# adr-arroyo/PointCloudComparator

Measured on AMD Instinct MI355X. Metric: nn_queries_per_sec, higher is better.
Workload: dtype f32; 1 GPU; C3: 10M x 10M XYZRGB (32-B stride), k=1 NN; step = index build over 10000000 references + 10000000 queries on each GPU (10000000 over 1 GPU); backend=none, engine=grid, references=10000000, queries_per_gpu=10000000, queries_total=10000000, point_stride_bytes=32

## Files before the change

pointcloudcomparator_amd/csrc/cellsort_mp.hip:

```cpp
#include "pcc_internal.hpp"
#include "grid_device.hpp"
#include "lane_ops.hpp"

namespace pcc {

constexpr int MP_T = 256;
constexpr unsigned int MP_F2 = 2048;
constexpr unsigned int MP_B2 = 128;
constexpr unsigned int MP_MAX_B1 = 256;
constexpr unsigned int MP_MAX_G = 512;
constexpr unsigned int MP_SLICE2 = 8192;
constexpr unsigned int MP_STAGE_BYTES = 32768;
constexpr unsigned int MP_WIN = 8;
#ifndef PCC_MP_STAGE_PTS
#define PCC_MP_STAGE_PTS 3072
#endif
#ifndef PCC_MP_STAGE_ORD
#define PCC_MP_STAGE_ORD 6144
#endif
constexpr unsigned int MP_FINE_STAGE_PTS = PCC_MP_STAGE_PTS, MP_FINE_STAGE_ORD = PCC_MP_STAGE_ORD;

struct MpPlan {
    unsigned int F1, F2, B1, G1, slice1;
};
static MpPlan mp_plan(unsigned int ncells_cap, unsigned int n) {
    MpPlan p;
    p.F2 = MP_F2;
    while ((unsigned long long)p.F2 * MP_B2 * MP_MAX_B1 < (unsigned long long)ncells_cap + 1) p.F2 *= 2;
    p.F1 = p.F2 * MP_B2;
    p.B1 = (ncells_cap + p.F1) / p.F1;
    p.G1 = (n + 16383) / 16384;
    if (p.G1 > MP_MAX_G) p.G1 = MP_MAX_G;
    if (p.G1 < 1) p.G1 = 1;
    p.slice1 = (n + p.G1 - 1) / p.G1;
    return p;
}

__device__ __forceinline__ unsigned int mp_cell(const float4& v, const GridParams& g, bool voxel) {
    return voxel ? voxel_id(v, g) : cell_id(v, g);
}
__device__ __forceinline__ unsigned int mp_cell(const uint2& v, const GridParams&, bool) { return v.x; }
__device__ __forceinline__ unsigned int mp_position(const float4& v) { return (unsigned int)__float_as_int(v.w); }
__device__ __forceinline__ unsigned int mp_position(const uint2& v) { return v.y; }
template <class E> __device__ __forceinline__ E mp_make(const float4& v, unsigned int cell);
template <> __device__ __forceinline__ float4 mp_make<float4>(const float4& v, unsigned int) { return v; }
template <> __device__ __forceinline__ uint2 mp_make<uint2>(const float4& v, unsigned int cell) {
    return make_uint2(cell, (unsigned int)__float_as_int(v.w));
}

__global__ void __launch_bounds__(MP_T)
k_mp_hist1(const float4* __restrict__ pts, unsigned int n, const GridDev* __restrict__ gd, unsigned int F1, unsigned int B1,
           unsigned int slice, unsigned int* __restrict__ H, unsigned int* __restrict__ zero, unsigned int n_zero) {
    for (unsigned int z = blockIdx.x * MP_T + threadIdx.x; z < n_zero; z += gridDim.x * MP_T) zero[z] = 0u;
    __shared__ unsigned int cnt[MP_MAX_B1];
    const GridParams g = gd->g;
    const bool voxel = gd->voxel != 0;
    for (unsigned int b = threadIdx.x; b < B1; b += MP_T) cnt[b] = 0;
    __syncthreads();
    const unsigned int beg = blockIdx.x * slice, end = min(n, beg + slice);
    for (unsigned int i0 = beg + threadIdx.x; i0 < end; i0 += 4 * MP_T) {
        float4 v[4];
#pragma unroll
        for (int u = 0; u < 4; ++u)
            if (i0 + u * MP_T < end) v[u] = pts[i0 + u * MP_T];
#pragma unroll
        for (int u = 0; u < 4; ++u)
            if (i0 + u * MP_T < end && __float_as_int(v[u].w) >= 0) atomicAdd(&cnt[mp_cell(v[u], g, voxel) / F1], 1u);
    }
    __syncthreads();
    for (unsigned int b = threadIdx.x; b < B1; b += MP_T) H[(size_t)b * gridDim.x + blockIdx.x] = cnt[b];
    if (blockIdx.x == 0 && threadIdx.x == 0) H[(size_t)B1 * gridDim.x] = 0;
}

template <class E>
__global__ void __launch_bounds__(MP_T)
k_mp_scatter1(const float4* __restrict__ pts, unsigned int n, const GridDev* __restrict__ gd, unsigned int F1, unsigned int B1,
              unsigned int slice, const unsigned int* __restrict__ H, E* __restrict__ out) {
    __shared__ unsigned int cur[MP_MAX_B1];
    const GridParams g = gd->g;
    const bool voxel = gd->voxel != 0;
    for (unsigned int b = threadIdx.x; b < B1; b += MP_T) cur[b] = H[(size_t)b * gridDim.x + blockIdx.x];
    __syncthreads();
    const unsigned int beg = blockIdx.x * slice, end = min(n, beg + slice);
    for (unsigned int i0 = beg + threadIdx.x; i0 < end; i0 += 4 * MP_T) {
        float4 v[4];
#pragma unroll
        for (int u = 0; u < 4; ++u)
            if (i0 + u * MP_T < end) v[u] = pts[i0 + u * MP_T];
#pragma unroll
        for (int u = 0; u < 4; ++u)
            if (i0 + u * MP_T < end && __float_as_int(v[u].w) >= 0) {
                const unsigned int c = mp_cell(v[u], g, voxel);
                out[atomicAdd(&cur[c / F1], 1u)] = mp_make<E>(v[u], c);
            }
    }
}

__global__ void __launch_bounds__(MP_T)
k_mp_hist1_cells(const unsigned int* __restrict__ cells, unsigned int n, unsigned int F1, unsigned int B1, unsigned int slice,
                 unsigned int* __restrict__ H, unsigned int* __restrict__ zero, unsigned int n_zero) {
    for (unsigned int z = blockIdx.x * MP_T + threadIdx.x; z < n_zero; z += gridDim.x * MP_T) zero[z] = 0u;
    __shared__ unsigned int cnt[MP_MAX_B1];
    for (unsigned int b = threadIdx.x; b < B1; b += MP_T) cnt[b] = 0;
    __syncthreads();
    const unsigned int beg = blockIdx.x * slice, end = min(n, beg + slice);
    for (unsigned int i0 = beg + threadIdx.x; i0 < end; i0 += 8 * MP_T) {
        unsigned int c[8];
#pragma unroll
        for (int u = 0; u < 8; ++u) c[u] = i0 + u * MP_T < end ? cells[i0 + u * MP_T] : 0xffffffffu;
#pragma unroll
        for (int u = 0; u < 8; ++u)
            if (c[u] != 0xffffffffu) atomicAdd(&cnt[c[u] / F1], 1u);
    }
    __syncthreads();
    for (unsigned int b = threadIdx.x; b < B1; b += MP_T) H[(size_t)b * gridDim.x + blockIdx.x] = cnt[b];
    if (blockIdx.x == 0 && threadIdx.x == 0) H[(size_t)B1 * gridDim.x] = 0;
}
__global__ void __launch_bounds__(MP_T)
k_mp_scatter1_cells(const unsigned int* __restrict__ cells, unsigned int n, unsigned int F1, unsigned int B1, unsigned int slice,
                    const unsigned int* __restrict__ H, uint2* __restrict__ out) {
    __shared__ unsigned int cur[MP_MAX_B1];
    for (unsigned int b = threadIdx.x; b < B1; b += MP_T) cur[b] = H[(size_t)b * gridDim.x + blockIdx.x];
    __syncthreads();
    const unsigned int beg = blockIdx.x * slice, end = min(n, beg + slice);
    for (unsigned int i0 = beg + threadIdx.x; i0 < end; i0 += 8 * MP_T) {
        unsigned int c[8];
#pragma unroll
        for (int u = 0; u < 8; ++u) c[u] = i0 + u * MP_T < end ? cells[i0 + u * MP_T] : 0xffffffffu;
#pragma unroll
        for (int u = 0; u < 8; ++u)
            if (c[u] != 0xffffffffu) out[atomicAdd(&cur[c[u] / F1], 1u)] = make_uint2(c[u], i0 + u * MP_T);
    }
}

constexpr unsigned int MP_TILE1 = 2048;
template <class E>
__global__ void __launch_bounds__(MP_T)
k_mp_scatter1_staged(const float4* __restrict__ pts, unsigned int n, const GridDev* __restrict__ gd, unsigned int F1, unsigned int B1,
                     unsigned int slice, const unsigned int* __restrict__ H, E* __restrict__ out) {
    constexpr int PER = MP_TILE1 / MP_T;
    __shared__ unsigned int cur[MP_MAX_B1], tcnt[MP_MAX_B1], tstart[MP_MAX_B1];
    __shared__ unsigned short sb[MP_TILE1];
    __shared__ __attribute__((aligned(16))) unsigned char stage_raw[MP_TILE1 * sizeof(E)];
    E* stage = reinterpret_cast<E*>(stage_raw);
    const GridParams g = gd->g;
    const bool voxel = gd->voxel != 0;
    for (unsigned int b = threadIdx.x; b < B1; b += MP_T) cur[b] = H[(size_t)b * gridDim.x + blockIdx.x];
    const unsigned int beg = blockIdx.x * slice, end = min(n, beg + slice);
    for (unsigned int t0 = beg; t0 < end; t0 += MP_TILE1) {
        for (unsigned int b = threadIdx.x; b < MP_MAX_B1; b += MP_T) tcnt[b] = 0;
        __syncthreads();
        float4 v[PER];
        unsigned int bk[PER], rk[PER];
#pragma unroll
        for (int u = 0; u < PER; ++u) {
            const unsigned int i = t0 + threadIdx.x + u * MP_T;
            v[u] = make_float4(0.f, 0.f, 0.f, __int_as_float(-1));
            if (i < end) v[u] = pts[i];
        }
#pragma unroll
        for (int u = 0; u < PER; ++u) {
            bk[u] = 0xffffffffu;
            rk[u] = 0;
            if (__float_as_int(v[u].w) >= 0) {
                bk[u] = mp_cell(v[u], g, voxel);
                rk[u] = atomicAdd(&tcnt[bk[u] / F1], 1u);
            }
        }
        __syncthreads();
        if (threadIdx.x < 64) {
            unsigned int c[4], sum = 0;
#pragma unroll
            for (int j = 0; j < 4; ++j) { c[j] = tcnt[4 * threadIdx.x + j]; sum += c[j]; }
            unsigned int ex = wave_incl_scan_add(sum) - sum;
#pragma unroll
            for (int j = 0; j < 4; ++j) { tstart[4 * threadIdx.x + j] = ex; ex += c[j]; }
        }
        __syncthreads();
#pragma unroll
        for (int u = 0; u < PER; ++u)
            if (bk[u] != 0xffffffffu) {
                const unsigned int b = bk[u] / F1, slot = tstart[b] + rk[u];
                stage[slot] = mp_make<E>(v[u], bk[u]);
                sb[slot] = (unsigned short)b;
            }
        __syncthreads();
        const unsigned int tile_n = tstart[MP_MAX_B1 - 1] + tcnt[MP_MAX_B1 - 1];
        for (unsigned int j = threadIdx.x; j < tile_n; j += MP_T) {
            const unsigned int b = sb[j];
            out[cur[b] + (j - tstart[b])] = stage[j];
        }
        __syncthreads();
        for (unsigned int b = threadIdx.x; b < MP_MAX_B1; b += MP_T) cur[b] += tcnt[b];
    }
}

__device__ __forceinline__ unsigned int mp_pair(unsigned int c, unsigned int F1, unsigned int F2) {
    return (c / F1) * MP_B2 + (c % F1) / F2;
}

template <bool PLACE, class E>
__global__ void __launch_bounds__(MP_T)
k_mp_level2(const E* __restrict__ in, const unsigned int* __restrict__ n_valid_ptr, const GridDev* __restrict__ gd,
            unsigned int F1, unsigned int F2, unsigned int* __restrict__ C, E* __restrict__ out) {
    constexpr unsigned int SLICE = PLACE ? MP_STAGE_BYTES / sizeof(E) : MP_SLICE2;
    __shared__ unsigned int cnt[MP_WIN * MP_B2];
    __shared__ __attribute__((aligned(16))) unsigned char stage_raw[PLACE ? MP_STAGE_BYTES : 16];
    E* stage = reinterpret_cast<E*>(stage_raw);
    const GridParams g = gd->g;
    const bool voxel = gd->voxel != 0;
    const unsigned int n = *n_valid_ptr;
    const unsigned int beg = blockIdx.x * SLICE, end = min(n, beg + SLICE);
    if (beg >= end) return;
    const unsigned int w0 = (mp_cell(in[beg], g, voxel) / F1) * MP_B2;
    for (unsigned int k = threadIdx.x; k < MP_WIN * MP_B2; k += MP_T) cnt[k] = 0;
    __syncthreads();
    for (unsigned int i0 = beg + threadIdx.x; i0 < end; i0 += 4 * MP_T) {
        E v[4];
#pragma unroll
        for (int u = 0; u < 4; ++u)
            if (i0 + u * MP_T < end) v[u] = in[i0 + u * MP_T];
#pragma unroll
        for (int u = 0; u < 4; ++u) {
            if (i0 + u * MP_T >= end) break;
            if (PLACE) stage[i0 + u * MP_T - beg] = v[u];
            const unsigned int pr = mp_pair(mp_cell(v[u], g, voxel), F1, F2);
            if (pr - w0 < MP_WIN * MP_B2) atomicAdd(&cnt[pr - w0], 1u);
            else if (!PLACE) atomicAdd(&C[pr], 1u);
            else out[atomicAdd(&C[pr], 1u)] = v[u];
        }
    }
    __syncthreads();
    for (unsigned int k = threadIdx.x; k < MP_WIN * MP_B2; k += MP_T) {
        const unsigned int c = cnt[k];
        if (c) {
            if (!PLACE) atomicAdd(&C[w0 + k], c);
            else cnt[k] = atomicAdd(&C[w0 + k], c);
        }
    }
    if (!PLACE) return;
    __syncthreads();
    for (unsigned int j = threadIdx.x; j < end - beg; j += MP_T) {
        const E v = stage[j];
        const unsigned int pr = mp_pair(mp_cell(v, g, voxel), F1, F2);
        if (pr - w0 < MP_WIN * MP_B2) out[atomicAdd(&cnt[pr - w0], 1u)] = v;
    }
}

__device__ __forceinline__ void mp_store_point(float4* out, unsigned int pos, const float4& v) { if (out) out[pos] = v; }
__device__ __forceinline__ void mp_store_point(float4*, unsigned int, const uint2&) {}

template <bool REFS, class E>
__global__ void __launch_bounds__(MP_T)
k_mp_fine(const E* __restrict__ in, const unsigned int* __restrict__ ends , const GridDev* __restrict__ gd,
          unsigned int F2, float4* __restrict__ out_pts, unsigned int* __restrict__ out_order,
          unsigned int* __restrict__ cell_start) {
    extern __shared__ __attribute__((aligned(16))) unsigned int lds[];
    unsigned int* cnt = lds;
    unsigned int* wsum = lds + F2;
    const GridParams g = gd->g;
    const bool voxel = gd->voxel != 0;
    const unsigned int ncells = (unsigned int)g.ncells;
    const unsigned int b = blockIdx.x;
    const unsigned int cell0 = b * F2;
    if (cell0 > ncells) return;
    const unsigned int beg = b ? ends[b - 1] : 0u, end = ends[b];
    if (!REFS && beg == end) return;
    for (unsigned int f = threadIdx.x; f < F2; f += MP_T) cnt[f] = 0;
    __syncthreads();
    for (unsigned int j0 = beg + threadIdx.x; j0 < end; j0 += 4 * MP_T) {
        E v[4];
#pragma unroll
        for (int u = 0; u < 4; ++u)
            if (j0 + u * MP_T < end) v[u] = in[j0 + u * MP_T];
#pragma unroll
        for (int u = 0; u < 4; ++u)
            if (j0 + u * MP_T < end) atomicAdd(&cnt[mp_cell(v[u], g, voxel) - cell0], 1u);
    }
    __syncthreads();
    const unsigned int per = (F2 + MP_T - 1) / MP_T;
    const unsigned int f0 = threadIdx.x * per, f1 = min(F2, f0 + per);
    unsigned int s = 0;
    for (unsigned int f = f0; f < f1; ++f) s += cnt[f];
    const unsigned int lane = threadIdx.x & 63, wave = threadIdx.x >> 6;
    const unsigned int inc = wave_incl_scan_add(s);
    if (lane == 63) wsum[wave] = inc;
    __syncthreads();
    unsigned int run = beg + inc - s;
    for (unsigned int w = 0; w < wave; ++w) run += wsum[w];
    for (unsigned int f = f0; f < f1; ++f) {
        const unsigned int c = cnt[f];
        cnt[f] = run;
        if (REFS && cell0 + f <= ncells) cell_start[cell0 + f] = run;
        run += c;
    }
    __syncthreads();
    const unsigned int stage_cap = out_pts ? MP_FINE_STAGE_PTS : MP_FINE_STAGE_ORD;
    const bool staged = end - beg <= stage_cap;
    float4* st_pts = reinterpret_cast<float4*>(lds + ((F2 + 4 + 3) & ~3u));
    unsigned int* st_ord = reinterpret_cast<unsigned int*>(st_pts + (out_pts ? MP_FINE_STAGE_PTS : 0));
    for (unsigned int j0 = beg + threadIdx.x; j0 < end; j0 += 4 * MP_T) {
        E v[4];
#pragma unroll
        for (int u = 0; u < 4; ++u)
            if (j0 + u * MP_T < end) v[u] = in[j0 + u * MP_T];
#pragma unroll
        for (int u = 0; u < 4; ++u) {
            if (j0 + u * MP_T >= end) break;
            const unsigned int pos = atomicAdd(&cnt[mp_cell(v[u], g, voxel) - cell0], 1u);
            if (staged) {
                mp_store_point(out_pts ? st_pts : nullptr, pos - beg, v[u]);
                if (out_order) st_ord[pos - beg] = mp_position(v[u]);
            } else {
                mp_store_point(out_pts, pos, v[u]);
                if (out_order) out_order[pos] = mp_position(v[u]);
            }
        }
    }
    if (staged) {
        __syncthreads();
        for (unsigned int i = threadIdx.x; i < end - beg; i += MP_T) {
            if (out_pts) out_pts[beg + i] = st_pts[i];
            if (out_order) out_order[beg + i] = st_ord[i];
        }
    }
}

int cell_sort_mp(pcc_index* ix, const float4* pts, size_t n_pts, bool refs, float4* out_pts, unsigned int* out_order,
                 unsigned int* cell_start, unsigned int** n_sorted_dev, const GridDev* gd_override,
                 unsigned int nc_cap_override) {
    hipStream_t s = ix->stream;
    const unsigned int n = (unsigned int)n_pts;
    const unsigned int ncap = gd_override ? nc_cap_override : ix->nc_cap;
    const MpPlan p = mp_plan(ncap, n);
    const GridDev* gd = gd_override ? gd_override : ix->d_grid.as<GridDev>();
    const unsigned int np = p.B1 * MP_B2;
    PCC_TRY(ix->mp_a.reserve((size_t)n * sizeof(float4) + 256));
    PCC_TRY(ix->mp_b.reserve((size_t)n * sizeof(float4) + 256));
    const size_t h_elems = (size_t)p.B1 * p.G1 + 1;
    PCC_TRY(ix->scratch_b.reserve(((h_elems + 3) & ~(size_t)3) * sizeof(unsigned int)));
    PCC_TRY(ix->mp_c.reserve(((size_t)np + 8) * sizeof(unsigned int)));
    unsigned int* H = ix->scratch_b.as<unsigned int>();
    unsigned int* C = ix->mp_c.as<unsigned int>();
    const unsigned int* cells = nullptr;
    if (!refs && !out_pts && !gd_override && pts == ix->q_packed.as<float4>() && ix->q_cells_n == n_pts && n_pts != 0)
        cells = ix->q_cells.as<unsigned int>();
    if (!refs) ix->q_cells_n = 0;
    if (cells)
        hipLaunchKernelGGL(k_mp_hist1_cells, dim3(p.G1), dim3(MP_T), 0, s, cells, n, p.F1, p.B1, p.slice1, H, C, np);
    else
    hipLaunchKernelGGL(k_mp_hist1, dim3(p.G1), dim3(MP_T), 0, s, pts, n, gd, p.F1, p.B1, p.slice1, H, C, np);
    PCC_HIP(hipGetLastError());
    PCC_TRY(launch_exclusive_scan(ix, s, H, h_elems, ix->scratch_a));
    unsigned int* n_valid = H + h_elems - 1;
    if (n_sorted_dev) *n_sorted_dev = n_valid;
    const size_t lds3 = (((size_t)p.F2 + 4 + 3) & ~(size_t)3) * sizeof(unsigned int) +
                        (out_pts ? (size_t)MP_FINE_STAGE_PTS * (sizeof(float4) + (out_order ? sizeof(unsigned int) : 0))
                                 : (size_t)MP_FINE_STAGE_ORD * sizeof(unsigned int));
    const unsigned int g2c = (n + MP_SLICE2 - 1) / MP_SLICE2;
    if (out_pts) {
        float4* t1 = ix->mp_a.as<float4>();
        float4* t2 = ix->mp_b.as<float4>();
        const unsigned int g2p = (n + MP_STAGE_BYTES / sizeof(float4) - 1) / (MP_STAGE_BYTES / sizeof(float4));
        if (ix->opt.sort_stage1)
            hipLaunchKernelGGL((k_mp_scatter1_staged<float4>), dim3(p.G1), dim3(MP_T), 0, s, pts, n, gd, p.F1, p.B1, p.slice1, H, t1);
        else
            hipLaunchKernelGGL((k_mp_scatter1<float4>), dim3(p.G1), dim3(MP_T), 0, s, pts, n, gd, p.F1, p.B1, p.slice1, H, t1);
        hipLaunchKernelGGL((k_mp_level2<false, float4>), dim3(g2c), dim3(MP_T), 0, s, t1, n_valid, gd, p.F1, p.F2, C, t2);
        PCC_TRY(launch_exclusive_scan(ix, s, C, np, ix->scratch_a));
        hipLaunchKernelGGL((k_mp_level2<true, float4>), dim3(g2p), dim3(MP_T), 0, s, t1, n_valid, gd, p.F1, p.F2, C, t2);
        if (refs)
            hipLaunchKernelGGL((k_mp_fine<true, float4>), dim3(np), dim3(MP_T), lds3, s, t2, C, gd, p.F2, out_pts, out_order, cell_start);
        else
            hipLaunchKernelGGL((k_mp_fine<false, float4>), dim3(np), dim3(MP_T), lds3, s, t2, C, gd, p.F2, out_pts, out_order, cell_start);
    } else {
        uint2* t1 = ix->mp_a.as<uint2>();
        uint2* t2 = ix->mp_b.as<uint2>();
        const unsigned int g2p = (n + MP_STAGE_BYTES / sizeof(uint2) - 1) / (MP_STAGE_BYTES / sizeof(uint2));
        if (cells)
            hipLaunchKernelGGL(k_mp_scatter1_cells, dim3(p.G1), dim3(MP_T), 0, s, cells, n, p.F1, p.B1, p.slice1, H, t1);
        else if (ix->opt.sort_stage1 == 2)
            hipLaunchKernelGGL((k_mp_scatter1_staged<uint2>), dim3(p.G1), dim3(MP_T), 0, s, pts, n, gd, p.F1, p.B1, p.slice1, H, t1);
        else
            hipLaunchKernelGGL((k_mp_scatter1<uint2>), dim3(p.G1), dim3(MP_T), 0, s, pts, n, gd, p.F1, p.B1, p.slice1, H, t1);
        hipLaunchKernelGGL((k_mp_level2<false, uint2>), dim3(g2c), dim3(MP_T), 0, s, t1, n_valid, gd, p.F1, p.F2, C, t2);
        PCC_TRY(launch_exclusive_scan(ix, s, C, np, ix->scratch_a));
        hipLaunchKernelGGL((k_mp_level2<true, uint2>), dim3(g2p), dim3(MP_T), 0, s, t1, n_valid, gd, p.F1, p.F2, C, t2);
        if (refs)
            hipLaunchKernelGGL((k_mp_fine<true, uint2>), dim3(np), dim3(MP_T), lds3, s, t2, C, gd, p.F2, out_pts, out_order, cell_start);
        else
            hipLaunchKernelGGL((k_mp_fine<false, uint2>), dim3(np), dim3(MP_T), lds3, s, t2, C, gd, p.F2, out_pts, out_order, cell_start);
    }
    PCC_HIP(hipGetLastError());
    return PCC_OK;
}

}
```

Measured before the change: 7.300 billion queries/s.

## Add wave-level and single-read paths for light buckets in fine cell sort

The fine cell-sort kernel now picks a path by bucket size. Buckets with at most `light` points are handled by one wave each, using 16-bit packed counters and a wave-local scan, with four such buckets per extra block. Mid-size buckets use a one-read block path that keeps points in registers and records each point's rank from the counting atomic, so the input is not read a second time. This is meant to cut per-bucket block overhead, barriers and repeated global reads on sparse buckets. The cost is extra blocks in the grid, more LDS reserved per block, and a lot more branching and code complexity.

```diff
diff --git a/pointcloudcomparator_amd/csrc/cellsort_mp.hip b/pointcloudcomparator_amd/csrc/cellsort_mp.hip
--- a/pointcloudcomparator_amd/csrc/cellsort_mp.hip
+++ b/pointcloudcomparator_amd/csrc/cellsort_mp.hip
@@ -1,6 +1,7 @@
 #include "pcc_internal.hpp"
 #include "grid_device.hpp"
 #include "lane_ops.hpp"
+#include <algorithm>
 
 namespace pcc {
 
@@ -251,21 +252,12 @@
 __device__ __forceinline__ void mp_store_point(float4*, unsigned int, const uint2&) {}
 
 template <bool REFS, class E>
-__global__ void __launch_bounds__(MP_T)
-k_mp_fine(const E* __restrict__ in, const unsigned int* __restrict__ ends , const GridDev* __restrict__ gd,
-          unsigned int F2, float4* __restrict__ out_pts, unsigned int* __restrict__ out_order,
-          unsigned int* __restrict__ cell_start) {
-    extern __shared__ __attribute__((aligned(16))) unsigned int lds[];
+__device__ __forceinline__ void mp_fine_block(unsigned int* lds, const E* __restrict__ in, unsigned int beg, unsigned int end, unsigned int cell0,
+                                              const GridParams& g, bool voxel, unsigned int F2, float4* __restrict__ out_pts,
+                                              unsigned int* __restrict__ out_order, unsigned int* __restrict__ cell_start) {
     unsigned int* cnt = lds;
     unsigned int* wsum = lds + F2;
-    const GridParams g = gd->g;
-    const bool voxel = gd->voxel != 0;
     const unsigned int ncells = (unsigned int)g.ncells;
-    const unsigned int b = blockIdx.x;
-    const unsigned int cell0 = b * F2;
-    if (cell0 > ncells) return;
-    const unsigned int beg = b ? ends[b - 1] : 0u, end = ends[b];
-    if (!REFS && beg == end) return;
     for (unsigned int f = threadIdx.x; f < F2; f += MP_T) cnt[f] = 0;
     __syncthreads();
     for (unsigned int j0 = beg + threadIdx.x; j0 < end; j0 += 4 * MP_T) {
@@ -323,6 +315,163 @@
             if (out_pts) out_pts[beg + i] = st_pts[i];
             if (out_order) out_order[beg + i] = st_ord[i];
         }
+    }
+}
+
+#ifndef PCC_MP_LIGHT_PTS
+#define PCC_MP_LIGHT_PTS 1024
+#endif
+#ifndef PCC_MP_LIGHT_ORD
+#define PCC_MP_LIGHT_ORD 1024
+#endif
+template <class E> struct MpWave;
+template <> struct MpWave<float4> {
+    typedef float4 Staged;
+    static constexpr unsigned int LIGHT = PCC_MP_LIGHT_PTS;
+    static __device__ __forceinline__ float4 staged(const float4& v) { return v; }
+    static __device__ __forceinline__ void store(float4* out_pts, unsigned int*, unsigned int pos, const float4& v) { out_pts[pos] = v; }
+};
+template <> struct MpWave<uint2> {
+    typedef unsigned int Staged;
+    static constexpr unsigned int LIGHT = PCC_MP_LIGHT_ORD;
+    static __device__ __forceinline__ unsigned int staged(const uint2& v) { return v.y; }
+    static __device__ __forceinline__ void store(float4*, unsigned int* out_order, unsigned int pos, unsigned int v) { out_order[pos] = v; }
+};
+template <class E> constexpr unsigned int mp_wave_words() {
+    return MP_F2 / 2 + MpWave<E>::LIGHT * (unsigned int)(sizeof(typename MpWave<E>::Staged) / sizeof(unsigned int));
+}
+static_assert(PCC_MP_LIGHT_PTS % 64 == 0 && PCC_MP_LIGHT_ORD % 64 == 0 && PCC_MP_LIGHT_PTS < 65536 && PCC_MP_LIGHT_ORD < 65536,
+              "a light bucket is whole rounds of a wave and fits a 16-bit counter");
+
+template <bool REFS, class E>
+__device__ __forceinline__ void mp_fine_wave(unsigned int* cnt , const E* __restrict__ in, unsigned int beg, unsigned int n,
+                                             unsigned int cell0, const GridParams& g, bool voxel, float4* __restrict__ out_pts,
+                                             unsigned int* __restrict__ out_order, unsigned int* __restrict__ cell_start) {
+    typedef MpWave<E> W;
+    constexpr unsigned int PER = W::LIGHT / 64;
+    const unsigned int ncells = (unsigned int)g.ncells;
+    const unsigned int lane = threadIdx.x & 63;
+    if (n == 0) {
+        for (unsigned int f = lane; f < MP_F2; f += 64)
+            if (cell0 + f <= ncells) cell_start[cell0 + f] = beg;
+        return;
+    }
+    unsigned short* cnt16 = reinterpret_cast<unsigned short*>(cnt);
+    typename W::Staged* stage = reinterpret_cast<typename W::Staged*>(cnt + MP_F2 / 2);
+    E v[PER];
+#pragma unroll
+    for (unsigned int u = 0; u < PER; ++u) v[u] = in[beg + min(lane + 64 * u, n - 1)];
+    for (unsigned int k = lane; k < MP_F2 / 8; k += 64) reinterpret_cast<uint4*>(cnt)[k] = make_uint4(0u, 0u, 0u, 0u);
+    wave_lds_sync();
+    unsigned int key[PER];
+#pragma unroll
+    for (unsigned int u = 0; u < PER; ++u)
+        if (lane + 64 * u < n) {
+            const unsigned int c = (mp_cell(v[u], g, voxel) - cell0) & (MP_F2 - 1), sh = 16 * (c & 1);
+            const unsigned int old = atomicAdd(&cnt[c >> 1], 1u << sh);
+            key[u] = c | ((old >> sh) & 0xffffu) << 16;
+        }
+    wave_lds_sync();
+    unsigned int base = 0;
+#pragma unroll 8
+    for (unsigned int step = 0; step < MP_F2 / 64; ++step) {
+        const unsigned int f = 64 * step + lane;
+        const unsigned int c = cnt16[f];
+        const unsigned int inc = wave_incl_scan_add(c);
+        const unsigned int first = base + inc - c;
+        cnt16[f] = (unsigned short)first;
+        if (REFS && cell0 + f <= ncells) cell_start[cell0 + f] = beg + first;
+        base += __builtin_amdgcn_readlane(inc, 63);
+    }
+    wave_lds_sync();
+#pragma unroll
+    for (unsigned int u = 0; u < PER; ++u)
+        if (lane + 64 * u < n) key[u] = cnt16[key[u] & 0xffffu] + (key[u] >> 16);
+#pragma unroll
+    for (unsigned int u = 0; u < PER; ++u)
+        if (lane + 64 * u < n) stage[key[u]] = W::staged(v[u]);
+    wave_lds_sync();
+    for (unsigned int i = lane; i < n; i += 64) W::store(out_pts, out_order, beg + i, stage[i]);
+}
+
+template <class E> constexpr unsigned int mp_once_cap() { return MP_T * MpWave<E>::LIGHT / 64; }
+template <class E> constexpr unsigned int mp_once_words() {
+    return MP_F2 + 4 + mp_once_cap<E>() * (unsigned int)(sizeof(typename MpWave<E>::Staged) / sizeof(unsigned int));
+}
+template <bool REFS, class E>
+__device__ __forceinline__ void mp_fine_once(unsigned int* lds, const E* __restrict__ in, unsigned int beg, unsigned int n, unsigned int cell0,
+                                             const GridParams& g, bool voxel, float4* __restrict__ out_pts,
+                                             unsigned int* __restrict__ out_order, unsigned int* __restrict__ cell_start) {
+    typedef MpWave<E> W;
+    constexpr unsigned int PER = W::LIGHT / 64;
+    unsigned int* cnt = lds;
+    unsigned int* wsum = lds + MP_F2;
+    typename W::Staged* stage = reinterpret_cast<typename W::Staged*>(lds + MP_F2 + 4);
+    const unsigned int ncells = (unsigned int)g.ncells;
+    E v[PER];
+#pragma unroll
+    for (unsigned int u = 0; u < PER; ++u) v[u] = in[beg + min(threadIdx.x + MP_T * u, n - 1)];
+    for (unsigned int f = threadIdx.x; f < MP_F2; f += MP_T) cnt[f] = 0;
+    __syncthreads();
+    unsigned int key[PER];
+#pragma unroll
+    for (unsigned int u = 0; u < PER; ++u)
+        if (threadIdx.x + MP_T * u < n) {
+            const unsigned int c = (mp_cell(v[u], g, voxel) - cell0) & (MP_F2 - 1);
+            key[u] = c | atomicAdd(&cnt[c], 1u) << 16;
+        }
+    __syncthreads();
+    constexpr unsigned int per = MP_F2 / MP_T;
+    const unsigned int f0 = threadIdx.x * per;
+    unsigned int s = 0;
+#pragma unroll
+    for (unsigned int f = f0; f < f0 + per; ++f) s += cnt[f];
+    const unsigned int lane = threadIdx.x & 63, wave = threadIdx.x >> 6;
+    const unsigned int inc = wave_incl_scan_add(s);
+    if (lane == 63) wsum[wave] = inc;
+    __syncthreads();
+    unsigned int run = inc - s;
+    for (unsigned int w = 0; w < wave; ++w) run += wsum[w];
+#pragma unroll
+    for (unsigned int f = f0; f < f0 + per; ++f) {
+        const unsigned int c = cnt[f];
+        cnt[f] = run;
+        if (REFS && cell0 + f <= ncells) cell_start[cell0 + f] = beg + run;
+        run += c;
+    }
+    __syncthreads();
+#pragma unroll
+    for (unsigned int u = 0; u < PER; ++u)
+        if (threadIdx.x + MP_T * u < n) key[u] = cnt[key[u] & 0xffffu] + (key[u] >> 16);
+#pragma unroll
+    for (unsigned int u = 0; u < PER; ++u)
+        if (threadIdx.x + MP_T * u < n) stage[key[u]] = W::staged(v[u]);
+    __syncthreads();
+    for (unsigned int i = threadIdx.x; i < n; i += MP_T) W::store(out_pts, out_order, beg + i, stage[i]);
+}
+static_assert(MP_T * PCC_MP_LIGHT_PTS / 64 < 65536 && MP_T * PCC_MP_LIGHT_ORD / 64 < 65536, "a rank of the one-read block form fits 16 bits");
+
+template <bool REFS, class E>
+__global__ void __launch_bounds__(MP_T)
+k_mp_fine(const E* __restrict__ in, const unsigned int* __restrict__ ends , const GridDev* __restrict__ gd,
+          unsigned int F2, unsigned int n_block, unsigned int light, float4* __restrict__ out_pts, unsigned int* __restrict__ out_order,
+          unsigned int* __restrict__ cell_start) {
+    extern __shared__ __attribute__((aligned(16))) unsigned int lds[];
+    const GridParams g = gd->g;
+    const bool voxel = gd->voxel != 0;
+    const unsigned int ncells = (unsigned int)g.ncells;
+    const bool block = blockIdx.x < n_block;
+    const unsigned int wave = __builtin_amdgcn_readfirstlane(threadIdx.x >> 6);
+    const unsigned int b = block ? blockIdx.x : 4 * (blockIdx.x - n_block) + wave;
+    const unsigned int cell0 = b * F2;
+    if (cell0 > ncells) return;
+    const unsigned int beg = b ? ends[b - 1] : 0u, end = ends[b];
+    if (!REFS && beg == end) return;
+    if (block) {
+        if (light == 0 || end - beg > mp_once_cap<E>()) mp_fine_block<REFS, E>(lds, in, beg, end, cell0, g, voxel, F2, out_pts, out_order, cell_start);
+        else if (end - beg > light) mp_fine_once<REFS, E>(lds, in, beg, end - beg, cell0, g, voxel, out_pts, out_order, cell_start);
+    } else if (end - beg <= light) {
+        mp_fine_wave<REFS, E>(lds + wave * mp_wave_words<E>(), in, beg, end - beg, cell0, g, voxel, out_pts, out_order, cell_start);
     }
 }
 
@@ -354,9 +503,14 @@
     PCC_TRY(launch_exclusive_scan(ix, s, H, h_elems, ix->scratch_a));
     unsigned int* n_valid = H + h_elems - 1;
     if (n_sorted_dev) *n_sorted_dev = n_valid;
-    const size_t lds3 = (((size_t)p.F2 + 4 + 3) & ~(size_t)3) * sizeof(unsigned int) +
-                        (out_pts ? (size_t)MP_FINE_STAGE_PTS * (sizeof(float4) + (out_order ? sizeof(unsigned int) : 0))
-                                 : (size_t)MP_FINE_STAGE_ORD * sizeof(unsigned int));
+    const size_t lds3_block = (((size_t)p.F2 + 4 + 3) & ~(size_t)3) * sizeof(unsigned int) +
+                              (out_pts ? (size_t)MP_FINE_STAGE_PTS * (sizeof(float4) + (out_order ? sizeof(unsigned int) : 0))
+                                       : (size_t)MP_FINE_STAGE_ORD * sizeof(unsigned int));
+    const unsigned int light = p.F2 != MP_F2 || (out_pts != nullptr) == (out_order != nullptr) ? 0u : out_pts ? MpWave<float4>::LIGHT : MpWave<uint2>::LIGHT;
+    const size_t lds3_wave = !light ? 0 : 4 * sizeof(unsigned int) * (out_pts ? mp_wave_words<float4>() : mp_wave_words<uint2>());
+    const size_t lds3_once = !light ? 0 : sizeof(unsigned int) * (out_pts ? mp_once_words<float4>() : mp_once_words<uint2>());
+    const size_t lds3 = std::max(lds3_block, std::max(lds3_wave, lds3_once));
+    const unsigned int g3 = np + (light ? np / 4 : 0u);
     const unsigned int g2c = (n + MP_SLICE2 - 1) / MP_SLICE2;
     if (out_pts) {
         float4* t1 = ix->mp_a.as<float4>();
@@ -370,9 +524,9 @@
         PCC_TRY(launch_exclusive_scan(ix, s, C, np, ix->scratch_a));
         hipLaunchKernelGGL((k_mp_level2<true, float4>), dim3(g2p), dim3(MP_T), 0, s, t1, n_valid, gd, p.F1, p.F2, C, t2);
         if (refs)
-            hipLaunchKernelGGL((k_mp_fine<true, float4>), dim3(np), dim3(MP_T), lds3, s, t2, C, gd, p.F2, out_pts, out_order, cell_start);
+            hipLaunchKernelGGL((k_mp_fine<true, float4>), dim3(g3), dim3(MP_T), lds3, s, t2, C, gd, p.F2, np, light, out_pts, out_order, cell_start);
         else
-            hipLaunchKernelGGL((k_mp_fine<false, float4>), dim3(np), dim3(MP_T), lds3, s, t2, C, gd, p.F2, out_pts, out_order, cell_start);
+            hipLaunchKernelGGL((k_mp_fine<false, float4>), dim3(g3), dim3(MP_T), lds3, s, t2, C, gd, p.F2, np, light, out_pts, out_order, cell_start);
     } else {
         uint2* t1 = ix->mp_a.as<uint2>();
         uint2* t2 = ix->mp_b.as<uint2>();
@@ -387,9 +541,9 @@
         PCC_TRY(launch_exclusive_scan(ix, s, C, np, ix->scratch_a));
         hipLaunchKernelGGL((k_mp_level2<true, uint2>), dim3(g2p), dim3(MP_T), 0, s, t1, n_valid, gd, p.F1, p.F2, C, t2);
         if (refs)
-            hipLaunchKernelGGL((k_mp_fine<true, uint2>), dim3(np), dim3(MP_T), lds3, s, t2, C, gd, p.F2, out_pts, out_order, cell_start);
+            hipLaunchKernelGGL((k_mp_fine<true, uint2>), dim3(g3), dim3(MP_T), lds3, s, t2, C, gd, p.F2, np, light, out_pts, out_order, cell_start);
         else
-            hipLaunchKernelGGL((k_mp_fine<false, uint2>), dim3(np), dim3(MP_T), lds3, s, t2, C, gd, p.F2, out_pts, out_order, cell_start);
+            hipLaunchKernelGGL((k_mp_fine<false, uint2>), dim3(g3), dim3(MP_T), lds3, s, t2, C, gd, p.F2, np, light, out_pts, out_order, cell_start);
     }
     PCC_HIP(hipGetLastError());
     return PCC_OK;
```

After: 7.450 billion queries/s, median of 6. 2.1% higher.
